# ramanathanlab/distllm

Hardware: NVIDIA H100
Metric: embedded chunks/sec @512-tok (higher is better)
Workload: dtype bf16

## Files before the change

### distllm_b200/csrc/attention.cuh

```cuda
#pragma once

#include "common.cuh"

namespace b2e {

constexpr int AT_KC = 64;
constexpr float AT_MASKED = -3.0e38f;

template <int D, int V>
struct AtCfg {
  static constexpr int COLS = D < 64 ? D : 64;
  static constexpr int ROW_BYTES = 2 * COLS;
  static constexpr int BOX = 64 * ROW_BYTES;
  static constexpr int NB = D / COLS;
  static constexpr int NWG = (V & 64) ? 4 : 2;
  static constexpr int QT = 64 * NWG;
  static constexpr int THREADS = 128 * NWG + (NWG == 4 ? 128 : 32);
  static constexpr int CONSUMER_REGS = 112, PRODUCER_REGS = 24;
  static constexpr int STAGES = D == 128 ? 3 : 4;
  static constexpr int Q_BYTES = NWG * NB * BOX;
  static constexpr int STAGE_BYTES = 2 * NB * BOX;
  static_assert(D == 32 || D == 64 || D == 128, "head_dim");
  static constexpr int BAR = Q_BYTES + STAGES * STAGE_BYTES;
  static constexpr int SMEM_BYTES = BAR + 256 + 1024;
  static_assert(SMEM_BYTES <= 232448, "shared memory");
};

__device__ long long* g_att_clock = nullptr;

__device__ __forceinline__ float poly_exp2(float x) {
  x = fmaxf(x, -126.0f);
  const float n = rintf(x);
  const float f = x - n;
  float p = fmaf(f, 9.6181291e-3f, 5.5504109e-2f);
  p = fmaf(f, p, 2.4022651e-1f);
  p = fmaf(f, p, 6.9314718e-1f);
  p = fmaf(f, p, 1.0f);
  return __int_as_float(__float_as_int(p) + (static_cast<int>(n) << 23));
}

template <int ROW_BYTES>
__device__ __forceinline__ uint64_t at_box_desc(uint32_t saddr) {
  if constexpr (ROW_BYTES == 128) return make_smem_desc_sw128(saddr);
  else return make_smem_desc_sw64(saddr);
}

__global__ void attn_prep_kernel(const int64_t* __restrict__ mask, float* __restrict__ bias,
                                 int* __restrict__ kv_chunks, int* __restrict__ plain_chunks, int B, int S,
                                 int S_pad) {
  const int b = blockIdx.x * (blockDim.x >> 5) + (threadIdx.x >> 5);
  if (b >= B) return;
  const int lane = threadIdx.x & 31;
  int last = 0;
  int first_off = S_pad;
  for (int j = lane; j < S_pad; j += 32) {
    float v = -INFINITY;
    bool on = false;
    if (j < S) {
      on = mask[static_cast<size_t>(b) * S + j] != 0;
      v = on ? 0.0f : AT_MASKED;
      if (on) last = j + 1;
    }
    if (!on) first_off = min(first_off, j);
    bias[static_cast<size_t>(b) * S_pad + j] = v;
  }
#pragma unroll
  for (int o = 16; o > 0; o >>= 1) {
    last = max(last, __shfl_xor_sync(0xffffffffu, last, o));
    first_off = min(first_off, __shfl_xor_sync(0xffffffffu, first_off, o));
  }
  if (lane == 0) {
    kv_chunks[b] = last > 0 ? (last + AT_KC - 1) / AT_KC : S_pad / AT_KC;
    plain_chunks[b] = first_off / AT_KC;
  }
}

template <int D, int MODE, int V>
__global__ void __launch_bounds__(AtCfg<D, V>::THREADS, 1)
attention_kernel(const __grid_constant__ CUtensorMap tm, const __grid_constant__ CUtensorMap tm_ctx,
                 const float* __restrict__ bias, const int* __restrict__ kv_chunks,
                 const int* __restrict__ plain_chunks, int B, int S, int S_pad, int heads, int kv_heads, int window,
                 float scale_log2e, const int* __restrict__ seq_cu, const int* __restrict__ seq_len,
                 h16* __restrict__ ctx) {
  using Cfg = AtCfg<D, V>;
  constexpr int NB = Cfg::NB;
  constexpr int COLS = Cfg::COLS, BOX = Cfg::BOX, RB = Cfg::ROW_BYTES;
  constexpr int NWG = Cfg::NWG;
  constexpr int POLY = (V >> 2) & 3;
  constexpr bool EPI_ROLE = (V & 128) != 0;
  constexpr bool STAMPS = (V & 256) != 0;
  static_assert(MODE == 0 || (V & ~(64 | 128)) == 0, "windowed / causal attention: warpgroups and epilogue role only");
  const int h = blockIdx.x % heads;
  const int b = (blockIdx.x / heads) % B;
  const int tile = static_cast<int>(gridDim.x / (heads * B)) - 1 - static_cast<int>(blockIdx.x / (heads * B));
  const int row0 = seq_cu != nullptr ? __ldg(seq_cu + b) : b * S;
  const int len = seq_len != nullptr ? __ldg(seq_len + b) : S;
  const int q0 = tile * Cfg::QT;
  if (q0 >= len) return;
  const int kvc = __ldg(kv_chunks + b);
  const int np = (V & 1) ? __ldg(plain_chunks + b) : 0;
  int lo = 0, hi = kvc;
  if (MODE == 1) {
    lo = max(0, q0 - window) / AT_KC;
    hi = min(kvc, (q0 + Cfg::QT - 1 + window) / AT_KC + 1);
  } else if (MODE == 2) {
    lo = window > 0 ? max(0, q0 - window + 1) / AT_KC : 0;
    hi = min(kvc, (q0 + Cfg::QT - 1) / AT_KC + 1);
  }
  if (lo >= hi) lo = hi - 1;

  extern __shared__ uint8_t smem_raw[];
  const uint32_t sb = (smem_u32(smem_raw) + 1023u) & ~1023u;
  const uint32_t q_bar = sb + Cfg::BAR;
  const uint32_t full_bar = q_bar + 8;
  const uint32_t empty_bar = full_bar + 8u * Cfg::STAGES;
  const uint32_t out_bar = empty_bar + 8u * Cfg::STAGES;
  const int warp = threadIdx.x >> 5;
  const int kvh = h / (heads / kv_heads);
  const int qcol = h * D, kcol = (heads + kvh) * D, vcol = (heads + kv_heads + kvh) * D;

  if (threadIdx.x == 0) {
    mbar_init(q_bar, 1);
    for (int s = 0; s < Cfg::STAGES; ++s) {
      mbar_init(full_bar + 8u * s, 1);
      mbar_init(empty_bar + 8u * s, NWG);
    }
    for (int w = 0; w < NWG; ++w) mbar_init(out_bar + 8u * w, 1);
    mbar_fence_init();
  }
  __syncthreads();

  if (warp >= 4 * NWG) {
    if constexpr (NWG == 4) asm volatile("setmaxnreg.dec.sync.aligned.u32 %0;" ::"n"(Cfg::PRODUCER_REGS));
    if (warp == 4 * NWG && elect_one()) {
      tma_prefetch_desc(&tm);
      mbar_expect_tx(q_bar, Cfg::Q_BYTES);
#pragma unroll
      for (int w = 0; w < NWG; ++w)
#pragma unroll
        for (int x = 0; x < NB; ++x)
          tma_load_2d(sb + (w * NB + x) * BOX, &tm, q_bar, qcol + COLS * x, row0 + q0 + 64 * w);
      int stage = 0;
      uint32_t phase = 0;
      for (int c = lo; c < hi; ++c) {
        mbar_wait(empty_bar + 8u * stage, phase ^ 1u);
        const uint32_t fb = full_bar + 8u * stage;
        const uint32_t dst = sb + Cfg::Q_BYTES + stage * Cfg::STAGE_BYTES;
        mbar_expect_tx(fb, Cfg::STAGE_BYTES);
#pragma unroll
        for (int x = 0; x < NB; ++x) {
          tma_load_2d(dst + x * BOX, &tm, fb, kcol + COLS * x, row0 + c * AT_KC);
          tma_load_2d(dst + (NB + x) * BOX, &tm, fb, vcol + COLS * x, row0 + c * AT_KC);
        }
        if (++stage == Cfg::STAGES) { stage = 0; phase ^= 1u; }
      }
      if constexpr (EPI_ROLE) {
        for (int w = 0; w < NWG; ++w) {
          mbar_wait(out_bar + 8u * w, 0);
          if (q0 + 64 * w + 64 > len) continue;
#pragma unroll
          for (int x = 0; x < NB; ++x)
            tma_store_2d(&tm_ctx, sb + (w * NB + x) * BOX, h * D + COLS * x, row0 + q0 + 64 * w);
        }
        tma_store_commit();
        tma_store_wait_all();
      }
    }
    return;
  }

  if constexpr (NWG == 4) asm volatile("setmaxnreg.inc.sync.aligned.u32 %0;" ::"n"(Cfg::CONSUMER_REGS));
  const int wg = warp >> 2;
  const int t = threadIdx.x & 127;
  const int quad = t & 3;
  const int qr = q0 + 64 * wg + 16 * (t >> 5) + ((t & 31) >> 2);
  const float* brow = bias + static_cast<size_t>(b) * S_pad;
  const uint32_t q_addr = sb + wg * NB * BOX;
  long long* clk = nullptr;
  int n_stamp = 0;
  if (STAMPS && blockIdx.x == 0 && threadIdx.x == 0) clk = g_att_clock;

  constexpr int OG = COLS / 8;
  float o[NB][4 * OG];
#pragma unroll
  for (int x = 0; x < NB; ++x)
#pragma unroll
    for (int i = 0; i < 4 * OG; ++i) o[x][i] = 0.0f;
  float m[2] = {-INFINITY, -INFINITY}, l[2] = {0.0f, 0.0f};

  mbar_wait(q_bar, 0);
  int stage = 0;
  uint32_t phase = 0;
  for (int c = lo; c < hi; ++c) {
    mbar_wait(full_bar + 8u * stage, phase);
    const uint32_t k_addr = sb + Cfg::Q_BYTES + stage * Cfg::STAGE_BYTES;
    const uint32_t v_addr = k_addr + NB * BOX;
    float s[32];
#pragma unroll
    for (int i = 0; i < 32; ++i) s[i] = 0.0f;
    wgmma_fence();
    constexpr int KB = COLS / 16;
#pragma unroll
    for (int kk = 0; kk < D / 16; ++kk)
      wgmma_64x64_ss<0>(s, at_box_desc<RB>(q_addr + (kk / KB) * BOX) + 2u * (kk % KB),
                        at_box_desc<RB>(k_addr + (kk / KB) * BOX) + 2u * (kk % KB), kk != 0);
    wgmma_commit();
    wgmma_wait<0>();
    reg_fence(s);
    if (STAMPS && clk != nullptr && n_stamp < 256) {
      clk[n_stamp] = clock64();
      clk[256 + n_stamp++] = 2 * c + 1;
    }

    const int kbase = c * AT_KC + 2 * quad;
    const bool plain = MODE == 0 && (V & 1) && c < np;
#pragma unroll
    for (int j = 0; j < 8; ++j) {
      const float2 bz = plain ? make_float2(0.0f, 0.0f) : *reinterpret_cast<const float2*>(brow + kbase + 8 * j);
#pragma unroll
      for (int e = 0; e < 4; ++e) {
        const int key = kbase + 8 * j + (e & 1);
        const int q = qr + 8 * (e >> 1);
        float x = fmaf(s[4 * j + e], scale_log2e, (e & 1) ? bz.y : bz.x);
        if (MODE == 1 && abs(q - key) > window) x = AT_MASKED;
        if (MODE == 2 && (key > q || (window > 0 && q - key >= window))) x = AT_MASKED;
        s[4 * j + e] = x;
      }
    }
    float alpha[2];
#pragma unroll
    for (int hf = 0; hf < 2; ++hf) {
      float mx = m[hf];
#pragma unroll
      for (int j = 0; j < 8; ++j) mx = fmaxf(mx, fmaxf(s[4 * j + 2 * hf], s[4 * j + 2 * hf + 1]));
      mx = fmaxf(mx, __shfl_xor_sync(0xffffffffu, mx, 1));
      mx = fmaxf(mx, __shfl_xor_sync(0xffffffffu, mx, 2));
      alpha[hf] = fast_exp2(m[hf] - mx);
      m[hf] = mx;
    }
    uint32_t p[4][4];
    float rs[2] = {0.0f, 0.0f};
#pragma unroll
    for (int j = 0; j < 8; ++j) {
#pragma unroll
      for (int hf = 0; hf < 2; ++hf) {
        const float x0 = s[4 * j + 2 * hf] - m[hf], x1 = s[4 * j + 2 * hf + 1] - m[hf];
        const int k0 = (2 * (j & 1) + hf) * 2;
        const float p0 = (k0 % 4) < POLY ? poly_exp2(x0) : fast_exp2(x0);
        const float p1 = ((k0 + 1) % 4) < POLY ? poly_exp2(x1) : fast_exp2(x1);
        rs[hf] += p0 + p1;
        p[j >> 1][(j & 1) * 2 + hf] = pack_h16x2(p0, p1);
      }
    }
#pragma unroll
    for (int hf = 0; hf < 2; ++hf) l[hf] = l[hf] * alpha[hf] + rs[hf];
#pragma unroll
    for (int x = 0; x < NB; ++x)
#pragma unroll
      for (int j = 0; j < OG; ++j) {
        o[x][4 * j + 0] *= alpha[0];
        o[x][4 * j + 1] *= alpha[0];
        o[x][4 * j + 2] *= alpha[1];
        o[x][4 * j + 3] *= alpha[1];
      }

#pragma unroll
    for (int x = 0; x < NB; ++x) reg_fence(o[x]);
    wgmma_fence();
#pragma unroll
    for (int kc = 0; kc < 4; ++kc)
#pragma unroll
      for (int x = 0; x < NB; ++x) {
        if constexpr (COLS == 64) wgmma_64x64_rs_tb(o[x], p[kc], make_smem_desc_sw128(v_addr + x * BOX + kc * 16 * 128));
        else wgmma_64x32_rs_tb(o[x], p[kc], make_smem_desc_sw64(v_addr + x * BOX + kc * 16 * 64));
      }
    wgmma_commit();
    wgmma_wait<0>();
#pragma unroll
    for (int x = 0; x < NB; ++x) reg_fence(o[x]);
    if (STAMPS && clk != nullptr && n_stamp < 256) {
      clk[n_stamp] = clock64();
      clk[256 + n_stamp++] = 2 * c + 2;
    }
    if (t == 0) mbar_arrive(empty_bar + 8u * stage);
    if (++stage == Cfg::STAGES) { stage = 0; phase ^= 1u; }
  }

  const bool staged = EPI_ROLE && q0 + 64 * wg + 64 <= len;
#pragma unroll
  for (int hf = 0; hf < 2; ++hf) {
    float tot = l[hf];
    tot += __shfl_xor_sync(0xffffffffu, tot, 1);
    tot += __shfl_xor_sync(0xffffffffu, tot, 2);
    const float inv = 1.0f / tot;
    const int q = qr + 8 * hf;
    if (staged) {
      const int r = q - q0 - 64 * wg;
      const int swz = RB == 128 ? (r & 7) : ((r >> 1) & 3);
#pragma unroll
      for (int x = 0; x < NB; ++x)
#pragma unroll
        for (int j = 0; j < OG; ++j) {
          const uint32_t off = r * RB + ((j ^ swz) << 4) + 4 * quad;
          *reinterpret_cast<uint32_t*>(smem_raw + (q_addr - smem_u32(smem_raw)) + x * BOX + off) =
              pack_h16x2(o[x][4 * j + 2 * hf] * inv, o[x][4 * j + 2 * hf + 1] * inv);
        }
      continue;
    }
    if (q >= len) continue;
    h16* orow = ctx + static_cast<size_t>(row0 + q) * (heads * D) + h * D + 2 * quad;
#pragma unroll
    for (int x = 0; x < NB; ++x)
#pragma unroll
      for (int j = 0; j < OG; ++j)
        *reinterpret_cast<uint32_t*>(orow + COLS * x + 8 * j) =
            pack_h16x2(o[x][4 * j + 2 * hf] * inv, o[x][4 * j + 2 * hf + 1] * inv);
  }
  if constexpr (EPI_ROLE) {
    fence_proxy_async_smem();
    asm volatile("bar.sync %0, 128;" ::"r"(1 + wg) : "memory");
    if (t == 0) mbar_arrive(out_bar + 8u * wg);
  }
}

}
```

### distllm_b200/csrc/b2e_api.cu

```cuda
#include "../../include/b2e.h"
#include "../../include/b2e_debug.h"

#include <cuda.h>
#include <cuda_runtime.h>

#include <cstdarg>
#include <cstdio>
#include <cstdlib>
#include <cstring>
#include <string>
#include <utility>
#include <vector>

#include "attention.cuh"
#include "binsearch.cuh"
#include "common.cuh"
#include "gemm.cuh"
#include "mistral_ops.cuh"
#include "pack.cuh"
#include "rowops.cuh"
#include "topk.cuh"
#include "topk_tc.cuh"

using namespace b2e;
// ... 190 lines not shown
int launch_gemm_epi(const CUtensorMap& ta, const GemmW& wb, void* out, const float* bias,
                    const h16* resid, int M, int N, int K, cudaStream_t st, const int* m_dev) {
  auto kern = gemm_h16_wgmma_kernel<EPI>;
  int smem = GemmPlan<false>::SMEM_BYTES;
  if (N % wb.bn != 0) return fail(B2E_ERR_INVALID, "gemm: N=%d is not a multiple of its W map's tile width %d", N, wb.bn);
  if (wb.absmax) {
    kern = gemm_h16_wgmma_kernel<EPI, false, true>;
    smem = GemmPlan<true>::SMEM_BYTES;
  } else if (wb.bn == 192) {
    if constexpr (epi_is_glu(EPI)) {
      return fail(B2E_ERR_INVALID, "gemm: the gated epilogues run 128-wide tiles only");
    } else {
      kern = gemm_h16_wgmma_kernel<EPI, false, false, 192>;
      smem = GemmPlan<false, 192>::SMEM_BYTES;
      if constexpr (EPI == EPI_BIAS || EPI == EPI_BIAS_GELU)
        if (g_gemm_profiling) kern = gemm_h16_wgmma_kernel<EPI, true, false, 192>;
    }
  } else if constexpr (EPI == EPI_BIAS || EPI == EPI_BIAS_GELU) {
    if (g_gemm_profiling) kern = gemm_h16_wgmma_kernel<EPI, true>;
  }
  int rc = ensure_smem_attr(kern, smem);
  if (rc) return rc;
  DeviceInfo dev;
  if ((rc = current_device_info(&dev))) return rc;
  const long long tiles = (long long)(N / wb.bn) * ((M + GEMM_BM - 1) / GEMM_BM);
  if (tiles > 0x7fffffffLL) return fail(B2E_ERR_INVALID, "gemm: %lld output tiles exceed one grid", tiles);
  CUtensorMap tm_out;
  if ((rc = make_tmap_h16(&tm_out, out, M, epi_is_glu(EPI) ? N / 2 : N, GEMM_BM))) return rc;
  const unsigned grid = (unsigned)(tiles < dev.sms ? tiles : dev.sms);
  kern<<<grid, GEMM_THREADS, smem, st>>>(ta, wb.tm, tm_out, static_cast<h16*>(out), bias, resid, M, N, K, m_dev,
                                         wb.absmax);
  CUDA_TRY(cudaGetLastError());
  return B2E_OK;
}

int launch_gemm(const CUtensorMap& ta, const GemmW& tb, void* out, const float* bias,
                const void* resid, int M, int N, int K, int epi, cudaStream_t st, const int* m_dev = nullptr) {
  const h16* r = static_cast<const h16*>(resid);
  switch (epi) {
    case B2E_EPI_BIAS: return launch_gemm_epi<EPI_BIAS>(ta, tb, out, bias, r, M, N, K, st, m_dev);
    case B2E_EPI_BIAS_GELU: return launch_gemm_epi<EPI_BIAS_GELU>(ta, tb, out, bias, r, M, N, K, st, m_dev);
    case B2E_EPI_BIAS_RESID: return launch_gemm_epi<EPI_BIAS_RESID>(ta, tb, out, bias, r, M, N, K, st, m_dev);
    case B2E_EPI_SWIGLU: return launch_gemm_epi<EPI_SWIGLU>(ta, tb, out, bias, r, M, N, K, st, m_dev);
    case B2E_EPI_GEGLU: return launch_gemm_epi<EPI_GEGLU>(ta, tb, out, bias, r, M, N, K, st, m_dev);
  }
  return fail(B2E_ERR_INVALID, "unknown epilogue %d", epi);
}

template <typename T>
struct DevBuf {
  T* p = nullptr;
  size_t cap = 0;
  operator T*() const { return p; }
  int grow(size_t n, uint64_t& gen, bool zero = false) {
    if (n <= cap) return B2E_OK;
    ++gen;
    release();
    CUDA_TRY(cudaMalloc(&p, n * sizeof(T)));
    if (zero) CUDA_TRY(cudaMemset(p, 0, n * sizeof(T)));
    cap = n;
    return B2E_OK;
  }
  void release() {
    cudaFree(p);
    p = nullptr;
    cap = 0;
  }
};

struct DeviceScratch {
  int device = -1;
  uint64_t gen = 0;
};

template <typename Scratch>
int follow_device(Scratch& s) {
  int dev = 0;
  CUDA_TRY(cudaGetDevice(&dev));
  if (dev != s.device) {
    s.release();
    s.device = dev;
    ++s.gen;
  }
  return B2E_OK;
}

struct AttnScratch : DeviceScratch {
  DevBuf<float> bias;
  DevBuf<int> kv_chunks;
  DevBuf<int> plain_chunks;
  int ensure(int B, int S_pad) {
    int rc;
    if ((rc = follow_device(*this)) || (rc = bias.grow((size_t)B * S_pad, gen)) || (rc = kv_chunks.grow(B, gen)) ||
        (rc = plain_chunks.grow(B, gen)))
      return rc;
    return B2E_OK;
  }
  void release() {
    bias.release();
    kv_chunks.release();
    plain_chunks.release();
  }
};

inline int attn_s_pad(int S) { return (S + AT_KC - 1) / AT_KC * AT_KC; }

int attention_prepare(AttnScratch& sc, const int64_t* mask, int B, int S, cudaStream_t st) {
  int rc;
  const int S_pad = attn_s_pad(S);
  if ((rc = sc.ensure(B, S_pad))) return rc;
  attn_prep_kernel<<<(B + 7) / 8, 256, 0, st>>>(mask, sc.bias, sc.kv_chunks, sc.plain_chunks, B, S, S_pad);
  CUDA_TRY(cudaGetLastError());
  return B2E_OK;
}

struct SeqLayout {
  const int* cu = nullptr;
  const int* len = nullptr;
  const int* t_real = nullptr;
  const int* tok_src = nullptr;
};

struct PackBuffers : DeviceScratch {
  DevBuf<int> len_raw, ok, len;
  DevBuf<int> cu;
  DevBuf<int> t_real;
  DevBuf<int> src;
  int ensure(int B, size_t tokens) {
    int rc;
    if ((rc = follow_device(*this)) || (rc = len_raw.grow(B, gen)) || (rc = ok.grow(B, gen)) ||
        (rc = len.grow(B, gen)) || (rc = cu.grow((size_t)B + 1, gen)) || (rc = t_real.grow(2, gen)) ||
        (rc = src.grow(tokens, gen)))
      return rc;
    return B2E_OK;
  }
  void release() {
    len_raw.release(); ok.release(); len.release(); cu.release(); t_real.release(); src.release();
  }
};

template <int D, int MODE, int V>
int launch_attention_kernel(const CUtensorMap& tm, const AttnScratch& sc, void* ctx, int B, int S, int heads,
                            int kv_heads, int window, cudaStream_t st, const SeqLayout& lay) {
  using Cfg = AtCfg<D, V>;
  auto kern = attention_kernel<D, MODE, V>;
  int rc = ensure_smem_attr(kern, Cfg::SMEM_BYTES);
  if (rc) return rc;
  CUtensorMap tm_ctx = {};
  if ((V & 128) && (rc = make_tmap_h16(&tm_ctx, ctx, (uint64_t)B * S, (uint64_t)heads * D, 64, Cfg::COLS))) return rc;
  const float scale_log2e = 1.4426950408889634f / sqrtf(static_cast<float>(D));
  const long long ctas = (long long)heads * B * ((S + Cfg::QT - 1) / Cfg::QT);
  if (ctas > 0x7fffffffLL)
    return fail(B2E_ERR_INVALID, "attention: %lld CTAs (heads=%d B=%d S=%d) exceed one grid", ctas, heads, B, S);
  kern<<<(unsigned)ctas, Cfg::THREADS, Cfg::SMEM_BYTES, st>>>(tm, tm_ctx, sc.bias, sc.kv_chunks, sc.plain_chunks, B, S,
                                                    attn_s_pad(S), heads, kv_heads, window, scale_log2e, lay.cu,
                                                    lay.len, static_cast<h16*>(ctx));
  CUDA_TRY(cudaGetLastError());
  return B2E_OK;
}

constexpr int AT_DEFAULT_VARIANT = 193;
int g_att3_variant = -1;
inline int att3_variant() {
  if (g_att3_variant < 0) {
    const char* e = getenv("B2E_ATT3");
    g_att3_variant = e ? atoi(e) : AT_DEFAULT_VARIANT;
  }
  return g_att3_variant;
}

int launch_attention(const CUtensorMap& tkv, const AttnScratch& sc, void* ctx, int B, int S, int heads,
                     cudaStream_t st, int window = 0, const SeqLayout& lay = SeqLayout()) {
  const int v = att3_variant();
#define B2E_ATT(MODE, V) launch_attention_kernel<64, MODE, V>(tkv, sc, ctx, B, S, heads, heads, window, st, lay)
  if (window > 0) {
    switch (v & 192) {
      case 0: return B2E_ATT(1, 0);
      case 64: return B2E_ATT(1, 64);
      case 128: return B2E_ATT(1, 128);
      case 192: return B2E_ATT(1, 192);
    }
    return fail(B2E_ERR_INVALID, "windowed attention: variant %d has no instantiation (bits 6-7 of the variant pick "
                "0, 64, 128 or 192)", v);
  }
  switch (v) {
    case 0: return B2E_ATT(0, 0);
    case 1: return B2E_ATT(0, 1);
    case 5: return B2E_ATT(0, 5);
    case 64: return B2E_ATT(0, 64);
    case 65: return B2E_ATT(0, 65);
    case 69: return B2E_ATT(0, 69);
    case 193: return B2E_ATT(0, 193);
    case 261: return B2E_ATT(0, 261);
    case 321: return B2E_ATT(0, 321);
  }
#undef B2E_ATT
  return fail(B2E_ERR_INVALID, "attention variant %d is not instantiated (0,1,5,64,65,69,193,261,321)", v);
}

int launch_attention_causal_d128(const void* qkv, AttnScratch& sc, void* ctx, int B, int S, int heads,
                                 int kv_heads, int window, cudaStream_t st, const SeqLayout& lay = SeqLayout()) {
  CUtensorMap tm;
  const int rc = make_tmap_h16(&tm, qkv, (uint64_t)B * S, (uint64_t)(heads + 2 * kv_heads) * 128, AT_KC);
  if (rc) return rc;
  return launch_attention_kernel<128, 2, 0>(tm, sc, ctx, B, S, heads, kv_heads, window, st, lay);
}

constexpr int AT_D32_VARIANT = 1;

int launch_attention_bidir(const CUtensorMap& tqkv, const AttnScratch& sc, void* ctx, int B, int S, int heads,
                           int head_dim, cudaStream_t st, const SeqLayout& lay = SeqLayout()) {
  if (head_dim == 32)
    return launch_attention_kernel<32, 0, AT_D32_VARIANT>(tqkv, sc, ctx, B, S, heads, heads, 0, st, lay);
  return launch_attention(tqkv, sc, ctx, B, S, heads, st, 0, lay);
}

#define DISPATCH_H(H, CALL)                                         \
  switch (H) {                                                      \
    case 256: { constexpr int HW = 256; CALL; break; }              \
    case 384: { constexpr int HW = 384; CALL; break; }              \
    case 512: { constexpr int HW = 512; CALL; break; }              \
    case 640: { constexpr int HW = 640; CALL; break; }              \
    case 768: { constexpr int HW = 768; CALL; break; }              \
    case 1024: { constexpr int HW = 1024; CALL; break; }            \
    case 1280: { constexpr int HW = 1280; CALL; break; }            \
    case 2048: { constexpr int HW = 2048; CALL; break; }            \
    case 2560: { constexpr int HW = 2560; CALL; break; }            \
    case 4096: { constexpr int HW = 4096; CALL; break; }            \
    default: return fail(B2E_ERR_INVALID, "hidden size %d not supported (need 256*{1,2,3,4,5,8,10,16}, 384 or 640)", (H)); \
  }

inline int row_blocks(int rows) { return (rows + ROW_WARPS - 1) / ROW_WARPS; }

int check_h(int H) {
  if (H == 384 || H == 640) return B2E_OK;
  if (H % 256 != 0) return fail(B2E_ERR_INVALID, "hidden size %d must be a multiple of 256, or 384 or 640", H);
  switch (H / 256) {
    case 1: case 2: case 3: case 4: case 5: case 8: case 10: case 16: return B2E_OK;
  }
  return fail(B2E_ERR_UNSUPPORTED, "hidden size %d not supported (built: 256 x {1,2,3,4,5,8,10,16}, 384, 640)", H);
}

struct PoolScratch : DeviceScratch {
  DevBuf<int> seq_len;
  DevBuf<int> kill;
  DevBuf<int> idx;
  DevBuf<float> w;
  DevBuf<float> count;
  DevBuf<float> part;
  int ensure(int B, int S, size_t part_elems) {
    int rc;
    if ((rc = follow_device(*this)) || (rc = seq_len.grow(B, gen)) || (rc = kill.grow(S, gen)) ||
        (rc = idx.grow(B, gen)) || (rc = w.grow((size_t)B * S, gen)) || (rc = count.grow(B, gen)) ||
        (rc = part.grow(part_elems, gen)))
      return rc;
    return B2E_OK;
  }
  void release() {
    seq_len.release(); kill.release(); idx.release(); w.release(); count.release(); part.release();
  }
};

inline int pool_nsplit(int S) {
  int n = (S + 63) / 64;
  return n < 1 ? 1 : (n > 16 ? 16 : n);
}

int launch_pool_weights(PoolScratch& ps, int64_t* mask, int B, int S, int pool_kind, int mutate,
                        cudaStream_t st) {
  seq_len_kernel<<<(B + 7) / 8, 256, 0, st>>>(mask, ps.seq_len, B, S);
  CUDA_TRY(cudaMemsetAsync(ps.kill, 0, sizeof(int) * S, st));
  kill_columns_kernel<<<(B + 255) / 256, 256, 0, st>>>(ps.seq_len, ps.kill, B, S);
  pool_weights_kernel<<<(B + 7) / 8, 256, 0, st>>>(mask, ps.seq_len, ps.kill, ps.w, ps.count, B, S,
                                                    pool_kind == B2E_POOL_MEAN_REF ? 1 : 0, mutate);
  CUDA_TRY(cudaGetLastError());
  return B2E_OK;
}

int launch_finalize(PoolScratch& ps, float* out, int B, int H, int nsplit, int l2, int round_mode,
                    cudaStream_t st) {
  pool_finalize_kernel<<<B, 256, (H + 32) * sizeof(float), st>>>(ps.part, ps.count, out, H, nsplit,
                                                                 l2, round_mode);
  CUDA_TRY(cudaGetLastError());
  return B2E_OK;
}

struct DeviceGuard {
  int prev = -1;
  DeviceGuard() {
    if (cudaGetDevice(&prev) != cudaSuccess) {
      cudaGetLastError();
      prev = -1;
    }
  }
  ~DeviceGuard() {
    if (prev >= 0) cudaSetDevice(prev);
  }
};

thread_local PoolScratch g_pool_scratch;
thread_local AttnScratch g_attn_scratch;
thread_local PackBuffers g_pack_scratch;

}

inline bool is_decoder(int arch) { return arch == B2E_ARCH_MISTRAL || arch == B2E_ARCH_QWEN3; }

namespace {
enum FinalNorm {
  NORM_POST_LN,
  NORM_ADD_LN,
  NORM_ADD_RMS,
};

using TrunkFn = int (*)(B2EEncoder* e, const int64_t* ids, const int64_t* mask, const int64_t* types, int B, int S,
                        cudaStream_t st, const SeqLayout& lay);

struct Family {
  int lead, stride;
  int wqkv, wo, w1, w2;
  bool w1_gated;
  int w1_epi;
  FinalNorm norm;
  int norm_g, norm_b;
  TrunkFn trunk;
};
const Family* family(int arch);
}

struct B2EEncoder {
  B2EModelDesc desc;
  const Family* fam = nullptr;
  int full_layers = 0;
  std::vector<const void*> w;
  int device = 0;
  int sms = 0;
  DevBuf<h16> hidden, qkv, ctx, tmp, ffn;
  DevBuf<float> xres, tok_scale;
  PoolScratch pool;
  AttnScratch attn;
  PackBuffers pack;
  std::vector<GemmW> tm_wqkv, tm_wo, tm_w1, tm_w2;
  DevBuf<int64_t> stage_in;
  DevBuf<float> stage_out;
  cudaStream_t own_stream = nullptr;
  float *rope_cos = nullptr, *rope_sin = nullptr;
  float *rope_cos2 = nullptr, *rope_sin2 = nullptr;

  const void* slot(int l, int k) const { return w[fam->lead + fam->stride * l + k]; }
  const float* final_norm(int k) const {
// ... 1255 lines not shown
```

Measured before the change: 5012.

## Add persistent attention CTAs with double-buffered Q/output and ping-pong turn scheduling

```diff
diff --git a/distllm_b200/csrc/attention.cuh b/distllm_b200/csrc/attention.cuh
--- a/distllm_b200/csrc/attention.cuh
+++ b/distllm_b200/csrc/attention.cuh
@@ -15,18 +15,28 @@
   static constexpr int NB = D / COLS;
   static constexpr int NWG = (V & 64) ? 4 : 2;
   static constexpr int QT = 64 * NWG;
-  static constexpr int THREADS = 128 * NWG + (NWG == 4 ? 128 : 32);
-  static constexpr int CONSUMER_REGS = 112, PRODUCER_REGS = 24;
+  static constexpr bool TURNS = (V & 16) != 0;
+  static constexpr bool PRODUCER_WG = NWG == 4 || TURNS;
+  static constexpr int THREADS = 128 * NWG + (PRODUCER_WG ? 128 : 32);
+  static constexpr int CONSUMER_REGS = TURNS ? 240 : 112, PRODUCER_REGS = 24;
+  static_assert(!TURNS || (NWG == 2 && D == 64), "turns: two consumer warpgroups, head_dim 64");
+  static constexpr bool PERSIST = (V & 32) != 0;
+  static_assert(!PERSIST || ((V & 128) && !TURNS), "persistent CTAs: epilogue role, no turns");
+  static constexpr int QBUF = PERSIST ? 2 : 1;
   static constexpr int STAGES = D == 128 ? 3 : 4;
   static constexpr int Q_BYTES = NWG * NB * BOX;
   static constexpr int STAGE_BYTES = 2 * NB * BOX;
   static_assert(D == 32 || D == 64 || D == 128, "head_dim");
-  static constexpr int BAR = Q_BYTES + STAGES * STAGE_BYTES;
+  static constexpr int KV_OFF = QBUF * Q_BYTES;
+  static constexpr int BAR = KV_OFF + STAGES * STAGE_BYTES;
   static constexpr int SMEM_BYTES = BAR + 256 + 1024;
   static_assert(SMEM_BYTES <= 232448, "shared memory");
 };
 
 __device__ long long* g_att_clock = nullptr;
+constexpr int AT_EV_START = -1;
+constexpr int AT_EV_Q = -2;
+constexpr int AT_EV_STORED = -3;
 
 __device__ __forceinline__ float poly_exp2(float x) {
   x = fmaxf(x, -126.0f);
@@ -37,6 +47,61 @@
   p = fmaf(f, p, 6.9314718e-1f);
   p = fmaf(f, p, 1.0f);
   return __int_as_float(__float_as_int(p) + (static_cast<int>(n) << 23));
+}
+
+template <int MODE, int V>
+__device__ __forceinline__ void at_softmax(float (&s)[32], float (&m)[2], float (&l)[2], float (&alpha)[2], int c,
+                                           int np, int qr, int quad, const float* brow, int window,
+                                           float scale_log2e) {
+  constexpr int POLY = (V >> 2) & 3;
+  const int kbase = c * AT_KC + 2 * quad;
+  const bool plain = MODE == 0 && (V & 1) && c < np;
+#pragma unroll
+  for (int j = 0; j < 8; ++j) {
+    const float2 bz = plain ? make_float2(0.0f, 0.0f) : *reinterpret_cast<const float2*>(brow + kbase + 8 * j);
+#pragma unroll
+    for (int e = 0; e < 4; ++e) {
+      const int key = kbase + 8 * j + (e & 1);
+      const int q = qr + 8 * (e >> 1);
+      float x = fmaf(s[4 * j + e], scale_log2e, (e & 1) ? bz.y : bz.x);
+      if (MODE == 1 && abs(q - key) > window) x = AT_MASKED;
+      if (MODE == 2 && (key > q || (window > 0 && q - key >= window))) x = AT_MASKED;
+      s[4 * j + e] = x;
+    }
+  }
+#pragma unroll
+  for (int hf = 0; hf < 2; ++hf) {
+    float mx = m[hf];
+#pragma unroll
+    for (int j = 0; j < 8; ++j) mx = fmaxf(mx, fmaxf(s[4 * j + 2 * hf], s[4 * j + 2 * hf + 1]));
+    mx = fmaxf(mx, __shfl_xor_sync(0xffffffffu, mx, 1));
+    mx = fmaxf(mx, __shfl_xor_sync(0xffffffffu, mx, 2));
+    alpha[hf] = fast_exp2(m[hf] - mx);
+    m[hf] = mx;
+  }
+  float rs[2] = {0.0f, 0.0f};
+#pragma unroll
+  for (int j = 0; j < 8; ++j) {
+#pragma unroll
+    for (int hf = 0; hf < 2; ++hf) {
+      const float x0 = s[4 * j + 2 * hf] - m[hf], x1 = s[4 * j + 2 * hf + 1] - m[hf];
+      const int k0 = (2 * (j & 1) + hf) * 2;
+      const float p0 = (k0 % 4) < POLY ? poly_exp2(x0) : fast_exp2(x0);
+      const float p1 = ((k0 + 1) % 4) < POLY ? poly_exp2(x1) : fast_exp2(x1);
+      rs[hf] += p0 + p1;
+      s[4 * j + 2 * hf] = p0;
+      s[4 * j + 2 * hf + 1] = p1;
+    }
+  }
+#pragma unroll
+  for (int hf = 0; hf < 2; ++hf) l[hf] = l[hf] * alpha[hf] + rs[hf];
+}
+
+__device__ __forceinline__ void at_pack_p(const float (&s)[32], uint32_t (&p)[4][4]) {
+#pragma unroll
+  for (int j = 0; j < 8; ++j)
+#pragma unroll
+    for (int hf = 0; hf < 2; ++hf) p[j >> 1][(j & 1) * 2 + hf] = pack_h16x2(s[4 * j + 2 * hf], s[4 * j + 2 * hf + 1]);
 }
 
 template <int ROW_BYTES>
@@ -75,6 +140,10 @@
   }
 }
 
+struct AtTile {
+  int h, b, row0, len, q0, lo, hi, np;
+};
+
 template <int D, int MODE, int V>
 __global__ void __launch_bounds__(AtCfg<D, V>::THREADS, 1)
 attention_kernel(const __grid_constant__ CUtensorMap tm, const __grid_constant__ CUtensorMap tm_ctx,
@@ -86,241 +155,304 @@
   constexpr int NB = Cfg::NB;
   constexpr int COLS = Cfg::COLS, BOX = Cfg::BOX, RB = Cfg::ROW_BYTES;
   constexpr int NWG = Cfg::NWG;
-  constexpr int POLY = (V >> 2) & 3;
   constexpr bool EPI_ROLE = (V & 128) != 0;
   constexpr bool STAMPS = (V & 256) != 0;
   static_assert(MODE == 0 || (V & ~(64 | 128)) == 0, "windowed / causal attention: warpgroups and epilogue role only");
-  const int h = blockIdx.x % heads;
-  const int b = (blockIdx.x / heads) % B;
-  const int tile = static_cast<int>(gridDim.x / (heads * B)) - 1 - static_cast<int>(blockIdx.x / (heads * B));
-  const int row0 = seq_cu != nullptr ? __ldg(seq_cu + b) : b * S;
-  const int len = seq_len != nullptr ? __ldg(seq_len + b) : S;
-  const int q0 = tile * Cfg::QT;
-  if (q0 >= len) return;
-  const int kvc = __ldg(kv_chunks + b);
-  const int np = (V & 1) ? __ldg(plain_chunks + b) : 0;
-  int lo = 0, hi = kvc;
-  if (MODE == 1) {
-    lo = max(0, q0 - window) / AT_KC;
-    hi = min(kvc, (q0 + Cfg::QT - 1 + window) / AT_KC + 1);
-  } else if (MODE == 2) {
-    lo = window > 0 ? max(0, q0 - window + 1) / AT_KC : 0;
-    hi = min(kvc, (q0 + Cfg::QT - 1) / AT_KC + 1);
-  }
-  if (lo >= hi) lo = hi - 1;
+  constexpr bool PERSIST = Cfg::PERSIST;
+  const long long t_start = STAMPS ? clock64() : 0;
+  const int tiles = (S + Cfg::QT - 1) / Cfg::QT;
+  const int n_tiles = tiles * heads * B;
+  const int tile_step = PERSIST ? static_cast<int>(gridDim.x) : n_tiles;
+  auto decode = [&](int idx) {
+    AtTile r;
+    r.h = MODE == 2 ? idx % heads : (idx / tiles) % heads;
+    const int b = MODE == 2 ? (idx / heads) % B : idx / (tiles * heads);
+    const int tile = MODE == 2 ? tiles - 1 - idx / (heads * B) : idx % tiles;
+    r.b = b;
+    r.row0 = seq_cu != nullptr ? __ldg(seq_cu + b) : b * S;
+    r.len = seq_len != nullptr ? __ldg(seq_len + b) : S;
+    r.q0 = tile * Cfg::QT;
+    const int kvc = __ldg(kv_chunks + b);
+    r.np = (V & 1) ? __ldg(plain_chunks + b) : 0;
+    r.lo = 0;
+    r.hi = kvc;
+    if (MODE == 1) {
+      r.lo = max(0, r.q0 - window) / AT_KC;
+      r.hi = min(kvc, (r.q0 + Cfg::QT - 1 + window) / AT_KC + 1);
+    } else if (MODE == 2) {
+      r.lo = window > 0 ? max(0, r.q0 - window + 1) / AT_KC : 0;
+      r.hi = min(kvc, (r.q0 + Cfg::QT - 1) / AT_KC + 1);
+    }
+    if (r.lo >= r.hi) r.lo = r.hi - 1;
+    return r;
+  };
+  if (!PERSIST) {
+    const int b = MODE == 2 ? (blockIdx.x / heads) % B : blockIdx.x / (tiles * heads);
+    const int tile = MODE == 2 ? tiles - 1 - static_cast<int>(blockIdx.x / (heads * B)) : blockIdx.x % tiles;
+    if (tile * Cfg::QT >= (seq_len != nullptr ? __ldg(seq_len + b) : S)) return;
+  }
 
   extern __shared__ uint8_t smem_raw[];
   const uint32_t sb = (smem_u32(smem_raw) + 1023u) & ~1023u;
   const uint32_t q_bar = sb + Cfg::BAR;
-  const uint32_t full_bar = q_bar + 8;
+  const uint32_t full_bar = q_bar + 8u * Cfg::QBUF;
   const uint32_t empty_bar = full_bar + 8u * Cfg::STAGES;
   const uint32_t out_bar = empty_bar + 8u * Cfg::STAGES;
   const int warp = threadIdx.x >> 5;
-  const int kvh = h / (heads / kv_heads);
-  const int qcol = h * D, kcol = (heads + kvh) * D, vcol = (heads + kv_heads + kvh) * D;
 
   if (threadIdx.x == 0) {
-    mbar_init(q_bar, 1);
+    for (int q = 0; q < Cfg::QBUF; ++q) mbar_init(q_bar + 8u * q, 1);
     for (int s = 0; s < Cfg::STAGES; ++s) {
       mbar_init(full_bar + 8u * s, 1);
       mbar_init(empty_bar + 8u * s, NWG);
     }
-    for (int w = 0; w < NWG; ++w) mbar_init(out_bar + 8u * w, 1);
+    for (int w = 0; w < Cfg::QBUF * NWG; ++w) mbar_init(out_bar + 8u * w, 1);
     mbar_fence_init();
   }
   __syncthreads();
 
   if (warp >= 4 * NWG) {
-    if constexpr (NWG == 4) asm volatile("setmaxnreg.dec.sync.aligned.u32 %0;" ::"n"(Cfg::PRODUCER_REGS));
+    if constexpr (Cfg::PRODUCER_WG) asm volatile("setmaxnreg.dec.sync.aligned.u32 %0;" ::"n"(Cfg::PRODUCER_REGS));
     if (warp == 4 * NWG && elect_one()) {
       tma_prefetch_desc(&tm);
-      mbar_expect_tx(q_bar, Cfg::Q_BYTES);
-#pragma unroll
-      for (int w = 0; w < NWG; ++w)
-#pragma unroll
-        for (int x = 0; x < NB; ++x)
-          tma_load_2d(sb + (w * NB + x) * BOX, &tm, q_bar, qcol + COLS * x, row0 + q0 + 64 * w);
-      int stage = 0;
+      auto store_tile = [&](const AtTile& tl, int n) {
+        const int buf = n % Cfg::QBUF;
+        for (int w = 0; w < NWG; ++w) {
+          mbar_wait(out_bar + 8u * (buf * NWG + w), (n / Cfg::QBUF) & 1);
+          if (tl.q0 + 64 * w + 64 > tl.len) continue;
+#pragma unroll
+          for (int x = 0; x < NB; ++x)
+            tma_store_2d(&tm_ctx, sb + buf * Cfg::Q_BYTES + (w * NB + x) * BOX, tl.h * D + COLS * x,
+                         tl.row0 + tl.q0 + 64 * w);
+        }
+        tma_store_commit();
+      };
+      int stage = 0, n = 0;
       uint32_t phase = 0;
-      for (int c = lo; c < hi; ++c) {
-        mbar_wait(empty_bar + 8u * stage, phase ^ 1u);
-        const uint32_t fb = full_bar + 8u * stage;
-        const uint32_t dst = sb + Cfg::Q_BYTES + stage * Cfg::STAGE_BYTES;
-        mbar_expect_tx(fb, Cfg::STAGE_BYTES);
-#pragma unroll
-        for (int x = 0; x < NB; ++x) {
-          tma_load_2d(dst + x * BOX, &tm, fb, kcol + COLS * x, row0 + c * AT_KC);
-          tma_load_2d(dst + (NB + x) * BOX, &tm, fb, vcol + COLS * x, row0 + c * AT_KC);
+      AtTile prev{};
+      for (int idx = blockIdx.x; idx < n_tiles; idx += tile_step) {
+        const AtTile tl = decode(idx);
+        if (tl.q0 >= tl.len) continue;
+        const int buf = n % Cfg::QBUF;
+        if (PERSIST && n >= 2) tma_store_wait_read<0>();
+        const int kvh = tl.h / (heads / kv_heads);
+        const int qcol = tl.h * D, kcol = (heads + kvh) * D, vcol = (heads + kv_heads + kvh) * D;
+        const uint32_t qb = q_bar + 8u * buf;
+        mbar_expect_tx(qb, Cfg::Q_BYTES);
+#pragma unroll
+        for (int w = 0; w < NWG; ++w)
+#pragma unroll
+          for (int x = 0; x < NB; ++x)
+            tma_load_2d(sb + buf * Cfg::Q_BYTES + (w * NB + x) * BOX, &tm, qb, qcol + COLS * x,
+                        tl.row0 + tl.q0 + 64 * w);
+        for (int c = tl.lo; c < tl.hi; ++c) {
+          mbar_wait(empty_bar + 8u * stage, phase ^ 1u);
+          const uint32_t fb = full_bar + 8u * stage;
+          const uint32_t dst = sb + Cfg::KV_OFF + stage * Cfg::STAGE_BYTES;
+          mbar_expect_tx(fb, Cfg::STAGE_BYTES);
+#pragma unroll
+          for (int x = 0; x < NB; ++x) {
+            tma_load_2d(dst + x * BOX, &tm, fb, kcol + COLS * x, tl.row0 + c * AT_KC);
+            tma_load_2d(dst + (NB + x) * BOX, &tm, fb, vcol + COLS * x, tl.row0 + c * AT_KC);
+          }
+          if (++stage == Cfg::STAGES) { stage = 0; phase ^= 1u; }
         }
-        if (++stage == Cfg::STAGES) { stage = 0; phase ^= 1u; }
+        if (EPI_ROLE && n >= 1) store_tile(prev, n - 1);
+        prev = tl;
+        ++n;
       }
       if constexpr (EPI_ROLE) {
-        for (int w = 0; w < NWG; ++w) {
-          mbar_wait(out_bar + 8u * w, 0);
-          if (q0 + 64 * w + 64 > len) continue;
-#pragma unroll
-          for (int x = 0; x < NB; ++x)
-            tma_store_2d(&tm_ctx, sb + (w * NB + x) * BOX, h * D + COLS * x, row0 + q0 + 64 * w);
-        }
-        tma_store_commit();
+        if (n >= 1) store_tile(prev, n - 1);
         tma_store_wait_all();
       }
     }
     return;
   }
 
-  if constexpr (NWG == 4) asm volatile("setmaxnreg.inc.sync.aligned.u32 %0;" ::"n"(Cfg::CONSUMER_REGS));
+  if constexpr (Cfg::PRODUCER_WG) asm volatile("setmaxnreg.inc.sync.aligned.u32 %0;" ::"n"(Cfg::CONSUMER_REGS));
   const int wg = warp >> 2;
   const int t = threadIdx.x & 127;
   const int quad = t & 3;
-  const int qr = q0 + 64 * wg + 16 * (t >> 5) + ((t & 31) >> 2);
-  const float* brow = bias + static_cast<size_t>(b) * S_pad;
-  const uint32_t q_addr = sb + wg * NB * BOX;
   long long* clk = nullptr;
   int n_stamp = 0;
-  if (STAMPS && blockIdx.x == 0 && threadIdx.x == 0) clk = g_att_clock;
-
+  if (STAMPS && blockIdx.x == 0 && t == 0 && g_att_clock != nullptr) clk = g_att_clock + 512 * wg;
+  auto stamp = [&](long long when, int event) {
+    if (STAMPS && clk != nullptr && n_stamp < 256) {
+      clk[n_stamp] = when;
+      clk[256 + n_stamp++] = event;
+    }
+  };
+  stamp(t_start, AT_EV_START);
+  auto k_addr_of = [&](int stage) { return sb + Cfg::KV_OFF + stage * Cfg::STAGE_BYTES; };
   constexpr int OG = COLS / 8;
-  float o[NB][4 * OG];
-#pragma unroll
-  for (int x = 0; x < NB; ++x)
-#pragma unroll
-    for (int i = 0; i < 4 * OG; ++i) o[x][i] = 0.0f;
-  float m[2] = {-INFINITY, -INFINITY}, l[2] = {0.0f, 0.0f};
-
-  mbar_wait(q_bar, 0);
-  int stage = 0;
+
+  int stage = 0, n = 0;
   uint32_t phase = 0;
-  for (int c = lo; c < hi; ++c) {
-    mbar_wait(full_bar + 8u * stage, phase);
-    const uint32_t k_addr = sb + Cfg::Q_BYTES + stage * Cfg::STAGE_BYTES;
-    const uint32_t v_addr = k_addr + NB * BOX;
-    float s[32];
-#pragma unroll
-    for (int i = 0; i < 32; ++i) s[i] = 0.0f;
-    wgmma_fence();
-    constexpr int KB = COLS / 16;
-#pragma unroll
-    for (int kk = 0; kk < D / 16; ++kk)
-      wgmma_64x64_ss<0>(s, at_box_desc<RB>(q_addr + (kk / KB) * BOX) + 2u * (kk % KB),
-                        at_box_desc<RB>(k_addr + (kk / KB) * BOX) + 2u * (kk % KB), kk != 0);
-    wgmma_commit();
-    wgmma_wait<0>();
-    reg_fence(s);
-    if (STAMPS && clk != nullptr && n_stamp < 256) {
-      clk[n_stamp] = clock64();
-      clk[256 + n_stamp++] = 2 * c + 1;
-    }
-
-    const int kbase = c * AT_KC + 2 * quad;
-    const bool plain = MODE == 0 && (V & 1) && c < np;
-#pragma unroll
-    for (int j = 0; j < 8; ++j) {
-      const float2 bz = plain ? make_float2(0.0f, 0.0f) : *reinterpret_cast<const float2*>(brow + kbase + 8 * j);
-#pragma unroll
-      for (int e = 0; e < 4; ++e) {
-        const int key = kbase + 8 * j + (e & 1);
-        const int q = qr + 8 * (e >> 1);
-        float x = fmaf(s[4 * j + e], scale_log2e, (e & 1) ? bz.y : bz.x);
-        if (MODE == 1 && abs(q - key) > window) x = AT_MASKED;
-        if (MODE == 2 && (key > q || (window > 0 && q - key >= window))) x = AT_MASKED;
-        s[4 * j + e] = x;
+  for (int idx = blockIdx.x; idx < n_tiles; idx += tile_step) {
+    const AtTile tl = decode(idx);
+    if (tl.q0 >= tl.len) continue;
+    const int lo = tl.lo, hi = tl.hi, np = tl.np, q0 = tl.q0, len = tl.len;
+    const int buf = n % Cfg::QBUF;
+    const int qr = q0 + 64 * wg + 16 * (t >> 5) + ((t & 31) >> 2);
+    const float* brow = bias + static_cast<size_t>(tl.b) * S_pad;
+    const uint32_t q_addr = sb + buf * Cfg::Q_BYTES + wg * NB * BOX;
+
+    float o[NB][4 * OG];
+#pragma unroll
+    for (int x = 0; x < NB; ++x)
+#pragma unroll
+      for (int i = 0; i < 4 * OG; ++i) o[x][i] = 0.0f;
+    float m[2] = {-INFINITY, -INFINITY}, l[2] = {0.0f, 0.0f};
+
+    auto issue_pv = [&](const uint32_t (&p)[4][4], uint32_t v_addr) {
+#pragma unroll
+      for (int x = 0; x < NB; ++x) reg_fence(o[x]);
+      wgmma_fence();
+#pragma unroll
+      for (int kc = 0; kc < 4; ++kc)
+#pragma unroll
+        for (int x = 0; x < NB; ++x) {
+          if constexpr (COLS == 64) wgmma_64x64_rs_tb(o[x], p[kc], make_smem_desc_sw128(v_addr + x * BOX + kc * 16 * 128));
+          else wgmma_64x32_rs_tb(o[x], p[kc], make_smem_desc_sw64(v_addr + x * BOX + kc * 16 * 64));
+        }
+      wgmma_commit();
+    };
+    auto issue_s = [&](float (&s)[32], uint32_t k_addr) {
+#pragma unroll
+      for (int i = 0; i < 32; ++i) s[i] = 0.0f;
+      wgmma_fence();
+      constexpr int KB = COLS / 16;
+#pragma unroll
+      for (int kk = 0; kk < D / 16; ++kk)
+        wgmma_64x64_ss<0>(s, at_box_desc<RB>(q_addr + (kk / KB) * BOX) + 2u * (kk % KB),
+                          at_box_desc<RB>(k_addr + (kk / KB) * BOX) + 2u * (kk % KB), kk != 0);
+      wgmma_commit();
+    };
+    auto rescale_o = [&](const float (&alpha)[2]) {
+#pragma unroll
+      for (int x = 0; x < NB; ++x)
+#pragma unroll
+        for (int j = 0; j < OG; ++j) {
+          o[x][4 * j + 0] *= alpha[0];
+          o[x][4 * j + 1] *= alpha[0];
+          o[x][4 * j + 2] *= alpha[1];
+          o[x][4 * j + 3] *= alpha[1];
+        }
+    };
+
+    mbar_wait(q_bar + 8u * buf, (n / Cfg::QBUF) & 1);
+    stamp(clock64(), AT_EV_Q);
+    if constexpr (!Cfg::TURNS) {
+      for (int c = lo; c < hi; ++c) {
+        mbar_wait(full_bar + 8u * stage, phase);
+        const uint32_t k_addr = k_addr_of(stage);
+        float s[32];
+        issue_s(s, k_addr);
+        wgmma_wait<0>();
+        reg_fence(s);
+        stamp(clock64(), 2 * c + 1);
+        float alpha[2];
+        at_softmax<MODE, V>(s, m, l, alpha, c, np, qr, quad, brow, window, scale_log2e);
+        uint32_t p[4][4];
+        at_pack_p(s, p);
+        rescale_o(alpha);
+        issue_pv(p, k_addr + NB * BOX);
+        wgmma_wait<0>();
+#pragma unroll
+        for (int x = 0; x < NB; ++x) reg_fence(o[x]);
+        stamp(clock64(), 2 * c + 2);
+        if (t == 0) mbar_arrive(empty_bar + 8u * stage);
+        if (++stage == Cfg::STAGES) { stage = 0; phase ^= 1u; }
       }
-    }
-    float alpha[2];
+    } else {
+      const int my_turn = 3 + wg, next_turn = 4 - wg;
+      auto end_turn = [&] { named_bar_arrive(next_turn, 256); };
+      if (wg == 1) end_turn();
+      float s[32], alpha[2];
+      uint32_t p[4][4];
+      mbar_wait(full_bar + 8u * stage, phase);
+      named_bar_sync(my_turn, 256);
+      issue_s(s, k_addr_of(stage));
+      end_turn();
+      wgmma_wait<0>();
+      reg_fence(s);
+      stamp(clock64(), 2 * lo + 1);
+      at_softmax<MODE, V>(s, m, l, alpha, lo, np, qr, quad, brow, window, scale_log2e);
+      at_pack_p(s, p);
+      for (int c = lo + 1; c < hi; ++c) {
+        const int prev = stage;
+        if (++stage == Cfg::STAGES) { stage = 0; phase ^= 1u; }
+        mbar_wait(full_bar + 8u * stage, phase);
+        named_bar_sync(my_turn, 256);
+        issue_s(s, k_addr_of(stage));
+        rescale_o(alpha);
+        issue_pv(p, k_addr_of(prev) + NB * BOX);
+        end_turn();
+        wgmma_wait<1>();
+        reg_fence(s);
+        stamp(clock64(), 2 * c + 1);
+        at_softmax<MODE, V>(s, m, l, alpha, c, np, qr, quad, brow, window, scale_log2e);
+        wgmma_wait<0>();
+#pragma unroll
+        for (int x = 0; x < NB; ++x) reg_fence(o[x]);
+#pragma unroll
+        for (int kc = 0; kc < 4; ++kc)
+#pragma unroll
+          for (int i = 0; i < 4; ++i) asm volatile("" : "+r"(p[kc][i])::"memory");
+        stamp(clock64(), 2 * c);
+        if (t == 0) mbar_arrive(empty_bar + 8u * prev);
+        at_pack_p(s, p);
+      }
+      named_bar_sync(my_turn, 256);
+      rescale_o(alpha);
+      issue_pv(p, k_addr_of(stage) + NB * BOX);
+      if (wg == 0) end_turn();
+      wgmma_wait<0>();
+#pragma unroll
+      for (int x = 0; x < NB; ++x) reg_fence(o[x]);
+      stamp(clock64(), 2 * hi);
+      if (t == 0) mbar_arrive(empty_bar + 8u * stage);
+      if (++stage == Cfg::STAGES) { stage = 0; phase ^= 1u; }
+    }
+
+    const bool staged = EPI_ROLE && q0 + 64 * wg + 64 <= len;
 #pragma unroll
     for (int hf = 0; hf < 2; ++hf) {
-      float mx = m[hf];
-#pragma unroll
-      for (int j = 0; j < 8; ++j) mx = fmaxf(mx, fmaxf(s[4 * j + 2 * hf], s[4 * j + 2 * hf + 1]));
-      mx = fmaxf(mx, __shfl_xor_sync(0xffffffffu, mx, 1));
-      mx = fmaxf(mx, __shfl_xor_sync(0xffffffffu, mx, 2));
-      alpha[hf] = fast_exp2(m[hf] - mx);
-      m[hf] = mx;
-    }
-    uint32_t p[4][4];
-    float rs[2] = {0.0f, 0.0f};
-#pragma unroll
-    for (int j = 0; j < 8; ++j) {
-#pragma unroll
-      for (int hf = 0; hf < 2; ++hf) {
-        const float x0 = s[4 * j + 2 * hf] - m[hf], x1 = s[4 * j + 2 * hf + 1] - m[hf];
-        const int k0 = (2 * (j & 1) + hf) * 2;
-        const float p0 = (k0 % 4) < POLY ? poly_exp2(x0) : fast_exp2(x0);
-        const float p1 = ((k0 + 1) % 4) < POLY ? poly_exp2(x1) : fast_exp2(x1);
-        rs[hf] += p0 + p1;
-        p[j >> 1][(j & 1) * 2 + hf] = pack_h16x2(p0, p1);
+      float tot = l[hf];
+      tot += __shfl_xor_sync(0xffffffffu, tot, 1);
+      tot += __shfl_xor_sync(0xffffffffu, tot, 2);
+      const float inv = 1.0f / tot;
+      const int q = qr + 8 * hf;
+      if (staged) {
+        const int r = q - q0 - 64 * wg;
+        const int swz = RB == 128 ? (r & 7) : ((r >> 1) & 3);
+#pragma unroll
+        for (int x = 0; x < NB; ++x)
+#pragma unroll
+          for (int j = 0; j < OG; ++j) {
+            const uint32_t off = r * RB + ((j ^ swz) << 4) + 4 * quad;
+            *reinterpret_cast<uint32_t*>(smem_raw + (q_addr - smem_u32(smem_raw)) + x * BOX + off) =
+                pack_h16x2(o[x][4 * j + 2 * hf] * inv, o[x][4 * j + 2 * hf + 1] * inv);
+          }
+        continue;
       }
-    }
-#pragma unroll
-    for (int hf = 0; hf < 2; ++hf) l[hf] = l[hf] * alpha[hf] + rs[hf];
-#pragma unroll
-    for (int x = 0; x < NB; ++x)
-#pragma unroll
-      for (int j = 0; j < OG; ++j) {
-        o[x][4 * j + 0] *= alpha[0];
-        o[x][4 * j + 1] *= alpha[0];
-        o[x][4 * j + 2] *= alpha[1];
-        o[x][4 * j + 3] *= alpha[1];
-      }
-
-#pragma unroll
-    for (int x = 0; x < NB; ++x) reg_fence(o[x]);
-    wgmma_fence();
-#pragma unroll
-    for (int kc = 0; kc < 4; ++kc)
-#pragma unroll
-      for (int x = 0; x < NB; ++x) {
-        if constexpr (COLS == 64) wgmma_64x64_rs_tb(o[x], p[kc], make_smem_desc_sw128(v_addr + x * BOX + kc * 16 * 128));
-        else wgmma_64x32_rs_tb(o[x], p[kc], make_smem_desc_sw64(v_addr + x * BOX + kc * 16 * 64));
-      }
-    wgmma_commit();
-    wgmma_wait<0>();
-#pragma unroll
-    for (int x = 0; x < NB; ++x) reg_fence(o[x]);
-    if (STAMPS && clk != nullptr && n_stamp < 256) {
-      clk[n_stamp] = clock64();
-      clk[256 + n_stamp++] = 2 * c + 2;
-    }
-    if (t == 0) mbar_arrive(empty_bar + 8u * stage);
-    if (++stage == Cfg::STAGES) { stage = 0; phase ^= 1u; }
-  }
-
-  const bool staged = EPI_ROLE && q0 + 64 * wg + 64 <= len;
-#pragma unroll
-  for (int hf = 0; hf < 2; ++hf) {
-    float tot = l[hf];
-    tot += __shfl_xor_sync(0xffffffffu, tot, 1);
-    tot += __shfl_xor_sync(0xffffffffu, tot, 2);
-    const float inv = 1.0f / tot;
-    const int q = qr + 8 * hf;
-    if (staged) {
-      const int r = q - q0 - 64 * wg;
-      const int swz = RB == 128 ? (r & 7) : ((r >> 1) & 3);
+      if (q >= len) continue;
+      h16* orow = ctx + static_cast<size_t>(tl.row0 + q) * (heads * D) + tl.h * D + 2 * quad;
 #pragma unroll
       for (int x = 0; x < NB; ++x)
 #pragma unroll
-        for (int j = 0; j < OG; ++j) {
-          const uint32_t off = r * RB + ((j ^ swz) << 4) + 4 * quad;
-          *reinterpret_cast<uint32_t*>(smem_raw + (q_addr - smem_u32(smem_raw)) + x * BOX + off) =
+        for (int j = 0; j < OG; ++j)
+          *reinterpret_cast<uint32_t*>(orow + COLS * x + 8 * j) =
               pack_h16x2(o[x][4 * j + 2 * hf] * inv, o[x][4 * j + 2 * hf + 1] * inv);
-        }
-      continue;
-    }
-    if (q >= len) continue;
-    h16* orow = ctx + static_cast<size_t>(row0 + q) * (heads * D) + h * D + 2 * quad;
-#pragma unroll
-    for (int x = 0; x < NB; ++x)
-#pragma unroll
-      for (int j = 0; j < OG; ++j)
-        *reinterpret_cast<uint32_t*>(orow + COLS * x + 8 * j) =
-            pack_h16x2(o[x][4 * j + 2 * hf] * inv, o[x][4 * j + 2 * hf + 1] * inv);
-  }
-  if constexpr (EPI_ROLE) {
-    fence_proxy_async_smem();
-    asm volatile("bar.sync %0, 128;" ::"r"(1 + wg) : "memory");
-    if (t == 0) mbar_arrive(out_bar + 8u * wg);
-  }
-}
-
-}
+    }
+    if constexpr (EPI_ROLE) {
+      fence_proxy_async_smem();
+      asm volatile("bar.sync %0, 128;" ::"r"(1 + wg) : "memory");
+      if (t == 0) mbar_arrive(out_bar + 8u * (buf * NWG + wg));
+    }
+    stamp(clock64(), AT_EV_STORED);
+    ++n;
+  }
+}
+
+}
diff --git a/distllm_b200/csrc/b2e_api.cu b/distllm_b200/csrc/b2e_api.cu
--- a/distllm_b200/csrc/b2e_api.cu
+++ b/distllm_b200/csrc/b2e_api.cu
@@ -366,14 +366,20 @@
   const long long ctas = (long long)heads * B * ((S + Cfg::QT - 1) / Cfg::QT);
   if (ctas > 0x7fffffffLL)
     return fail(B2E_ERR_INVALID, "attention: %lld CTAs (heads=%d B=%d S=%d) exceed one grid", ctas, heads, B, S);
-  kern<<<(unsigned)ctas, Cfg::THREADS, Cfg::SMEM_BYTES, st>>>(tm, tm_ctx, sc.bias, sc.kv_chunks, sc.plain_chunks, B, S,
+  unsigned grid = (unsigned)ctas;
+  if constexpr (Cfg::PERSIST) {
+    DeviceInfo dev;
+    if ((rc = current_device_info(&dev))) return rc;
+    if (ctas > dev.sms) grid = (unsigned)dev.sms;
+  }
+  kern<<<grid, Cfg::THREADS, Cfg::SMEM_BYTES, st>>>(tm, tm_ctx, sc.bias, sc.kv_chunks, sc.plain_chunks, B, S,
                                                     attn_s_pad(S), heads, kv_heads, window, scale_log2e, lay.cu,
                                                     lay.len, static_cast<h16*>(ctx));
   CUDA_TRY(cudaGetLastError());
   return B2E_OK;
 }
 
-constexpr int AT_DEFAULT_VARIANT = 193;
+constexpr int AT_DEFAULT_VARIANT = 225;
 int g_att3_variant = -1;
 inline int att3_variant() {
   if (g_att3_variant < 0) {
@@ -404,12 +410,15 @@
     case 64: return B2E_ATT(0, 64);
     case 65: return B2E_ATT(0, 65);
     case 69: return B2E_ATT(0, 69);
+    case 17: return B2E_ATT(0, 17);
     case 193: return B2E_ATT(0, 193);
+    case 225: return B2E_ATT(0, 225);
     case 261: return B2E_ATT(0, 261);
+    case 273: return B2E_ATT(0, 273);
     case 321: return B2E_ATT(0, 321);
   }
 #undef B2E_ATT
-  return fail(B2E_ERR_INVALID, "attention variant %d is not instantiated (0,1,5,64,65,69,193,261,321)", v);
+  return fail(B2E_ERR_INVALID, "attention variant %d is not instantiated (0,1,5,17,64,65,69,193,225,261,273,321)", v);
 }
 
 int launch_attention_causal_d128(const void* qkv, AttnScratch& sc, void* ctx, int B, int S, int heads,
```

New measurement: 5143 (median of 6 runs). 2.6% higher.
